# Soham4001A/F16_JSB

Hardware: AMD Instinct MI355X
Metric: env-steps/sec at 65 536 envs, 1/2/4/8 MI355X; HBM GB/s fraction (higher is better)
Workload: dtype f32

## Files before the change

f16_jsb_amd/csrc/f16_device.h:

```cpp
#pragma once
#include <hip/hip_runtime.h>
#include <stdint.h>

#include "../../include/f16env.h"
#include "f16_tables.h"

namespace f16 {

enum DebugBits {
  DBG_STATE_INDEX = 1,
  DBG_WINDOW_POS = 2,
  DBG_DONE_LIST = 4,
  DBG_TABLE_SEGMENT = 8,
  DBG_RESET_INDEX = 16,
  DBG_RING_SLOT = 32,
  DBG_FRAME_INDEX = 64,
};
#ifdef F16_DEBUG_CHECKS
__device__ unsigned int g_f16_violations;
#define F16_CHECK(cond, bit)                                   \
  do {                                                         \
    if (!(cond)) atomicOr(&::f16::g_f16_violations, (bit));    \
  } while (0)
#else
// ... 156 lines not shown
  const float T2 = 2.0f * __builtin_fmaf(q1, q3, -(q0 * q2));
  const float T5 = 2.0f * __builtin_fmaf(q2, q3, q0 * q1);
  const float T8 = __builtin_fmaf(q3, q3, __builtin_fmaf(-q2, q2, __builtin_fmaf(-q1, q1, q0 * q0)));
  const float we = (float)0.00007292115;
  pqr[0] = __builtin_fmaf(-T2, we, wI[0]);
  pqr[1] = __builtin_fmaf(-T5, we, wI[1]);
  pqr[2] = __builtin_fmaf(-T8, we, wI[2]);
}
__device__ __forceinline__ float ground_speed(float vx, float vy, float vz, float rx, float ry, float rz) {
  const float vv = vx * vx + vy * vy + vz * vz;
  const float vr = vx * rx + vy * ry + vz * rz;
  const float rr = rx * rx + ry * ry + rz * rz;
  return __builtin_amdgcn_sqrtf(fmaxf(vv - vr * vr * __builtin_amdgcn_rcpf(rr), 0.0f));
}
__device__ __forceinline__ void latch_from_state(Lane& L) {
  float pqr[3];
  pqr_aero(L.q, L.wI, pqr);
  L.lx[F16L_P_AERO] = pqr[0]; L.lx[F16L_Q_AERO] = pqr[1]; L.lx[F16L_R_AERO] = pqr[2];
  const double w = 0.00007292115;
  L.lx[F16L_VG_FPS] = ground_speed((float)(L.vI[0] + w * L.rI[1]), (float)(L.vI[1] - w * L.rI[0]), (float)L.vI[2],
                                   (float)L.rI[0], (float)L.rI[1], (float)L.rI[2]);
}

template <bool NT = false>
__device__ __forceinline__ void st16(float4* p, float4 v) {
  if (NT) {
    typedef float v4f __attribute__((ext_vector_type(4)));
    __builtin_nontemporal_store(__builtin_bit_cast(v4f, v), reinterpret_cast<v4f*>(p));
  } else {
    *p = v;
  }
}

template <bool GUST>
__device__ __forceinline__ void lane_unpack(const float4 (&c)[NCOL], float4 w, float4 g, Lane& L) {
  L.rI[0] = f2d(c[0].x, c[0].y); L.rI[1] = f2d(c[0].z, c[0].w);
  L.rI[2] = f2d(c[1].x, c[1].y); L.vI[0] = f2d(c[1].z, c[1].w);
  L.vI[1] = f2d(c[2].x, c[2].y); L.vI[2] = f2d(c[2].z, c[2].w);
  L.epa = f2d(c[3].x, c[3].y); L.ep_ret = f2d(c[3].z, c[3].w);
  L.ndv1[0] = c[4].x; L.ndv1[1] = c[4].y; L.ndv1[2] = c[4].z; L.dv2[0] = c[4].w;
  L.dv2[1] = c[5].x; L.dv2[2] = c[5].y; L.aI[0] = c[5].z; L.aI[1] = c[5].w;
  L.aI[2] = c[6].x; L.aIp[0] = c[6].y; L.aIp[1] = c[6].z; L.aIp[2] = c[6].w;
  L.q[0] = c[7].x; L.q[1] = c[7].y; L.q[2] = c[7].z; L.q[3] = c[7].w;
  L.wI[0] = c[8].x; L.wI[1] = c[8].y; L.wI[2] = c[8].z; L.wId[0] = c[8].w;
  L.wId[1] = c[9].x; L.wId[2] = c[9].y; L.ba[0] = 0.0f; L.ba[1] = c[9].z; L.ba[2] = c[9].w;
  L.tef = c[10].x; L.ail = c[10].y; L.ele = c[10].z; L.rud = c[10].w;
  L.lef = c[11].x; L.sb = c[11].y; L.pri = c[11].z; L.prp = c[11].w;
  L.ppi = c[12].x; L.pyi = c[12].y; L.pyp = c[12].z; L.ppp = 0.0f;
  L.n2 = without_sign_flag(c[12].w); L.n1 = 0.0f;
  L.lx[F16L_ALPHA] = c[13].x; L.lx[F16L_BETA] = c[13].y; L.lx[F16L_MACH] = c[13].z; L.lx[F16L_VC_KTS] = c[13].w;
  L.last_d = without_sign_flag(c[14].x); L.step = __float_as_int(c[14].y);
  L.lx[F16L_NPY] = c[14].z; L.lx[F16L_NPZ] = c[14].w;
  L.goal[0] = c[15].x; L.goal[1] = c[15].y; L.goal[2] = c[15].z; L.ep_count = __float_as_int(c[15].w);
  L.flags = (sign_flag(c[12].w) ? LANE_FLAG_AUG : 0) | (sign_flag(c[14].x) ? LANE_FLAG_FRESH : 0);
  latch_from_state(L);
#pragma unroll
  for (int j = 0; j < 3; ++j) {
    L.wst[j] = GUST ? (&w.x)[j] : 0.0f;
    L.gust[j] = GUST ? (&g.x)[j] : 0.0f;
    L.wind[j] = L.wst[j] + L.gust[j];
  }
}
template <bool GUST = false>
__device__ __forceinline__ void lane_fetch(const SoA& s, int64_t k, float4 (&c)[NCOL], float4& w, float4& g) {
  const int64_t n = s.n;
  const float4* p = s.c + k;
#pragma unroll
  for (int j = 0; j < NCOL; ++j, p += n) c[j] = *p;
  w = make_float4(0.f, 0.f, 0.f, 0.f);
  g = w;
  if (GUST) {
    w = *p;
    g = *(p + n);
  }
}
template <bool GUST = false>
__device__ __forceinline__ void lane_load(const SoA& s, int64_t k, Lane& L) {
  float4 c[NCOL], w, g;
  lane_fetch<GUST>(s, k, c, w, g);
  lane_unpack<GUST>(c, w, g, L);
}
__device__ __forceinline__ void lane_load_lds(const float4* cols, Lane& L) {
  float4 c[NCOL];
#pragma unroll
  for (int j = 0; j < NCOL; ++j) c[j] = cols[j];
  const float4 z = make_float4(0.f, 0.f, 0.f, 0.f);
  lane_unpack<false>(c, z, z, L);
}

template <bool GUST = false, int PART = 0, bool NT = false>
__device__ __forceinline__ void lane_store(const SoA& s, int64_t k, const Lane& L, bool with15 = true) {
  const int64_t n = s.n;
  float4 c[NCOL];
  c[0] = make_float4(dlo(L.rI[0]), dhi(L.rI[0]), dlo(L.rI[1]), dhi(L.rI[1]));
  c[1] = make_float4(dlo(L.rI[2]), dhi(L.rI[2]), dlo(L.vI[0]), dhi(L.vI[0]));
  c[2] = make_float4(dlo(L.vI[1]), dhi(L.vI[1]), dlo(L.vI[2]), dhi(L.vI[2]));
  c[3] = make_float4(dlo(L.epa), dhi(L.epa), dlo(L.ep_ret), dhi(L.ep_ret));
  c[4] = make_float4(L.ndv1[0], L.ndv1[1], L.ndv1[2], L.dv2[0]);
  c[5] = make_float4(L.dv2[1], L.dv2[2], L.aI[0], L.aI[1]);
  c[6] = make_float4(L.aI[2], L.aIp[0], L.aIp[1], L.aIp[2]);
  c[7] = make_float4(L.q[0], L.q[1], L.q[2], L.q[3]);
  c[8] = make_float4(L.wI[0], L.wI[1], L.wI[2], L.wId[0]);
  c[9] = make_float4(L.wId[1], L.wId[2], L.ba[1], L.ba[2]);
  c[10] = make_float4(L.tef, L.ail, L.ele, L.rud);
  c[11] = make_float4(L.lef, L.sb, L.pri, L.prp);
  c[12] = make_float4(L.ppi, L.pyi, L.pyp, with_sign_flag(L.n2, (L.flags & LANE_FLAG_AUG) != 0));
// ... 8 lines not shown
      if (j != 15 || with15) st16<NT>(p, c[j]);
  if (GUST && PART != 2) {
    st16<NT>(p, make_float4(L.wst[0], L.wst[1], L.wst[2], 0.0f));
    st16<NT>(p + n, make_float4(L.gust[0], L.gust[1], L.gust[2], 0.0f));
  }
}

struct Seg {
  int i;
  float f;
};
__device__ __forceinline__ float rcpf(float x) { return __builtin_amdgcn_rcpf(x); }
__device__ __forceinline__ float fsqrt(float x) { return __builtin_amdgcn_sqrtf(x); }
__device__ __forceinline__ float fdiv(float a, float b) { return a * __builtin_amdgcn_rcpf(b); }

template <int N>
__device__ __forceinline__ Seg bracket(const float (&bp)[N], const float* pairs, float x) {
#ifdef F16_BRACKET_CMP
  int i = 1;
#pragma unroll
  for (int k = 1; k < N - 1; ++k) i += (bp[k] < x) ? 1 : 0;
#else
  uint32_t c = 0;
#pragma unroll
  for (int k = 1; k < N - 1; ++k) c += __float_as_uint(bp[k] - x) >> 31;
  const int i = 1 + (int)c;
#endif
  F16_CHECK(i >= 1 && i <= N - 1, DBG_TABLE_SEGMENT);
  const float2 p = reinterpret_cast<const float2*>(pairs)[i - 1];
  float f = (x - p.x) * p.y;
  f = __builtin_amdgcn_fmed3f(f, 0.0f, 1.0f);
  return {i, f};
}
template <int N>
__device__ __forceinline__ Seg bracket_guess(const float* pairs, float x, float u) {
  static_assert(N >= 3, "guess bracket needs an interior breakpoint");
  const int g = (int)__builtin_amdgcn_fmed3f(u, 0.0f, (float)(N - 3));
  const float2* P = reinterpret_cast<const float2*>(pairs);
  const float2 p0 = P[g], p1 = P[g + 1];
  const bool up = x > p1.x;
  const float lo = up ? p1.x : p0.x, iv = up ? p1.y : p0.y;
  const int i = g + 1 + (up ? 1 : 0);
  F16_CHECK(i >= 1 && i <= N - 1, DBG_TABLE_SEGMENT);
  float f = (x - lo) * iv;
  f = __builtin_amdgcn_fmed3f(f, 0.0f, 1.0f);
  return {i, f};
}
template <int N>
constexpr double guess_h(const float (&bp)[N]) { return ((double)bp[N - 1] - (double)bp[0]) / (N - 1); }
template <int N>
constexpr bool guess_ok_uniform(const float (&bp)[N]) {
  const double h = guess_h(bp), x0 = (double)bp[0] + 0.5 * h;
  for (int k = 1; k <= N - 3; ++k) {
    const double b = x0 + k * h;
    if (!((double)bp[k] + 1e-5 < b && b < (double)bp[k + 1] - 1e-5)) return false;
  }
  return true;
}
template <int N>
__device__ __forceinline__ Seg bracket_g_uniform(const float (&bp)[N], const float* pairs, float x) {
  const double h = guess_h(bp);
  const float ginv = (float)(1.0 / h), c0 = (float)(-((double)bp[0] + 0.5 * h) / h);
  return bracket_guess<N>(pairs, x, __builtin_fmaf(x, ginv, c0));
}
__device__ __forceinline__ float machu_u(float x) {
  x = fminf(x, 4.0f);
// ... 493 lines not shown
    L.n2 = 60.0f + tp * 40.0f;
    L.n1 = 30.0f + tp * 70.0f;
    L.flags = (aug_cmd > 0.0f) ? (L.flags | LANE_FLAG_AUG) : (L.flags & ~LANE_FLAG_AUG);
  } else {
    const float nn = fminf((L.n2 - 60.0f) * (1.0f / 40.0f) + 0.1f, 1.0f);
    const float u = 1.0f - nn;
    const float spool = (90.0f / 3.36f) * rcpf(1.0f + 3.0f * u * u * u + (1.0f - sigma));
    L.n2 = seekf(L.n2, 60.0f + tp * 40.0f, spool, spool * 3.0f, dt);
    L.n1 = seekf(L.n1, 30.0f + tp * 70.0f, spool, spool * 2.4f, dt);
  }
  const float n2n = (L.n2 - 60.0f) * (1.0f / 40.0f);
  float thrust = idle + mil * n2n * n2n;
  if (!(L.flags & LANE_FLAG_AUG)) thrust *= (1.0f - 0.03f);
  if (aug_cmd > 0.0f) {
    L.flags |= LANE_FLAG_AUG;
    const float tdiff = 29000.0f * ev[2] - thrust;
    thrust += tdiff * aug_cmd;
  } else {
    L.flags &= ~LANE_FLAG_AUG;
  }
  return thrust;
}

struct AeroIn {
  float qbar, alpha, beta, mach, p, q, r, bi2vel, ci2vel, kclge;
  float de, da, dr, dlef, flap, dsb;
};
__device__ __forceinline__ void aero(const AeroIn& a, const float* T, float* F6) {
#ifdef F16_GUESS_BRACKET
  static_assert(guess_ok_uniform(BP_alpha_bp) && guess_ok_uniform(BP_beta13_bp) && machu_guess_ok(),
                "guess-bracket crossings must lie inside their segments");
  const Seg sa = bracket_g_uniform(BP_alpha_bp, T + OFF_pair_alpha, a.alpha);
#else
  const Seg sa = bracket(BP_alpha_bp, T + OFF_pair_alpha, a.alpha);
#endif
  float A[F16_N_A1D];
  {
    const float* r0 = T + (OFF_alpha1d + __umul24((unsigned)(sa.i - 1), 2u * F16_N_A1D));
#pragma unroll
    for (int k = 0; k < F16_N_A1D / 2; ++k) {
      const f2v r = blend2(sa.f, ld2(r0 + 2 * k), ld2(r0 + F16_N_A1D + 2 * k));
      A[2 * k] = r.x;
      A[2 * k + 1] = r.y;
    }
  }
  const Seg se = bracket(BP_de_bp, T + OFF_pair_de, a.de);
  float ADE[3];
  {
    const float* p0 = T + (OFF_ade + __umul24(__umul24((unsigned)(sa.i - 1), F16_N_DE) + (unsigned)(se.i - 1), 6u));
    const float* p1 = p0 + 6;
    const f2v c1 = blend2(sa.f, ld2(p0), ld2(p0 + 2)), c2 = blend2(sa.f, ld2(p1), ld2(p1 + 2));
    const f2v r = blend2(se.f, c1, c2 - c1);
    ADE[0] = r.x; ADE[1] = r.y;
    const f2v t1 = ld2(p0 + 4), t2 = ld2(p1 + 4);
    const float d1 = blend(sa.f, t1.x, t1.y), d2 = blend(sa.f, t2.x, t2.y);
    ADE[2] = d1 + se.f * (d2 - d1);
  }
#ifdef F16_GUESS_BRACKET
  const Seg sb13 = bracket_g_uniform(BP_beta13_bp, T + OFF_pair_beta13, a.beta);
#else
  const Seg sb13 = bracket(BP_beta13_bp, T + OFF_pair_beta13, a.beta);
#endif
  float AB13[2];
  {
    const float* p0 = T + (OFF_ab13 + 4u * (__umul24((unsigned)(sa.i - 1), F16_N_B13) + (unsigned)(sb13.i - 1)));
    const float* p1 = p0 + 4;
    const f2v c1 = blend2(sa.f, ld2(p0), ld2(p0 + 2)), c2 = blend2(sa.f, ld2(p1), ld2(p1 + 2));
    const f2v r = blend2(sb13.f, c1, c2 - c1);
    AB13[0] = r.x; AB13[1] = r.y;
  }
  static_assert(beta7_is_even_beta13(), "beta7 grid must be the even beta13 breakpoints");
  Seg sb7;
  {
    sb7.i = 1 + ((sb13.i - 1) >> 1);
    const float2 p = reinterpret_cast<const float2*>(T + OFF_pair_beta7)[sb7.i - 1];
    sb7.f = __builtin_amdgcn_fmed3f((a.beta - p.x) * p.y, 0.0f, 1.0f);
  }
  float AB7[4];
  {
    const float* p0 = T + (OFF_ab7 + 8u * (__umul24((unsigned)(sa.i - 1), F16_N_B7) + (unsigned)(sb7.i - 1)));
    const float* p1 = p0 + 8;
#pragma unroll
    for (int k = 0; k < 4; k += 2) {
      const f2v c1 = blend2(sa.f, ld2(p0 + k), ld2(p0 + k + 4)), c2 = blend2(sa.f, ld2(p1 + k), ld2(p1 + k + 4));
      const f2v r = blend2(sb7.f, c1, c2 - c1);
      AB7[k] = r.x; AB7[k + 1] = r.y;
    }
  }
#ifdef F16_GUESS_BRACKET
  const Seg sm = bracket_guess<13>(T + OFF_pair_machu, a.mach, machu_u(a.mach));
#else
  const Seg sm = bracket(BP_machu, T + OFF_pair_machu, a.mach);
#endif
  float MU[MACHU_NT];
  {
    const float* r0 = T + (OFF_machu_v + __umul24((unsigned)(sm.i - 1), 2u * MACHU_NT));
#pragma unroll
    for (int k = 0; k + 1 < MACHU_NT; k += 2) {
      const f2v r = blend2(sm.f, ld2(r0 + 2 * k), ld2(r0 + 2 * k + 2));
      MU[k] = r.x; MU[k + 1] = r.y;
    }
    if (MACHU_NT & 1) {
      const f2v t = ld2(r0 + 2 * MACHU_NT - 2);
      MU[MACHU_NT - 1] = blend(sm.f, t.x, t.y);
    }
  }
  const float CDmach = MU[MU_CDmach], CYb_M = MU[MU_CYb_M], Clb_M = MU[MU_Clb_M];
  const float Clda_M = MU[MU_Clda_M], Cldr_M = MU[MU_Cldr_M], Cma_M = MU[MU_Cma_M];
  const float Cnb_M = MU[MU_Cnb_M], Cnda_M = MU[MU_Cnda_M], Cndr_M = MU[MU_Cndr_M];

  const float qS = a.qbar * S_W;
  const float qc = a.q * a.ci2vel, pb = a.p * a.bi2vel, rb = a.r * a.bi2vel;
  const float D = qS * (ADE[ADE_CDDh] + CDmach + a.dlef * A[A1D_CDDlef] + a.flap * 0.08f +
                        0.0f * 0.027f + a.dsb * A[A1D_CDDsb] + qc * A[A1D_CDq] +
                        qc * a.dlef * A[A1D_CDq_Dlef]);
  const float Y = qS * (a.beta * -1.146f + a.beta * CYb_M + a.da * -0.0226f + a.dr * 0.086f +
                        pb * A[A1D_CYp] + rb * A[A1D_CYr]);
  const float Lf = qS * (a.kclge * ADE[ADE_CLDh] + a.dlef * a.kclge * A[A1D_CLDlef] +
                         a.flap * a.kclge * 0.35f + a.kclge * a.dsb * A[A1D_CLDsb] +
                         qc * a.kclge * A[A1D_CLq] + qc * a.dsb * A[A1D_CLq_Dsb]);
  const float qSb = qS * B_W, qSc = qS * CBAR;
  const float Lm = qSb * (AB13[AB13_Clb] + a.beta * Clb_M + pb * A[A1D_Clp] + rb * A[A1D_Clr] +
                          a.da * AB7[AB7_Clda] + a.alpha * a.da * Clda_M + a.alpha * a.dr * Cldr_M +
                          a.dr * AB7[AB7_Cldr]);
  const float Mm = qSc * (ADE[ADE_CmDh] + a.alpha * Cma_M + a.dsb * A[A1D_CmDsb] + qc * A[A1D_Cmq]);
  const float Nm = qSb * (AB13[AB13_Cnb] + a.beta * Cnb_M + pb * A[A1D_Cnp] + rb * A[A1D_Cnr] +
                          a.da * Cnda_M + a.da * AB7[AB7_Cnda] + a.dr * AB7[AB7_Cndr] +
                          a.alpha * a.dr * Cndr_M);
  F6[0] = D; F6[1] = Y; F6[2] = Lf; F6[3] = Lm; F6[4] = Mm; F6[5] = Nm;
}

template <bool LOWREG = false, bool WIND = true>
__device__ __forceinline__ void frame(Lane& L, const float* cmd, double& ce, double& se, const AltRef& A,
                                      const float* T, const ModelConsts& C, bool ic F16_STAMP_ARG) {
  const float dt = C.dt_f;
  const FcsTab tb = fcs_tables(L, T);
  if (!ic) {
    const float hx = C.half_dt * L.wI[0], hy = C.half_dt * L.wI[1], hz = C.half_dt * L.wI[2];
    const float a2 = hx * hx + hy * hy + hz * hz;
    float na2 = __builtin_fmaf(-hz, hz, __builtin_fmaf(-hx, hx, -(hy * hy)));
    if constexpr (!LOWREG) asm("" : "+v"(na2));
    float ca, sa;
    if constexpr (LOWREG) {
      ca = 1.0f - a2 * (0.5f - a2 * (1.0f / 24.0f - a2 * (1.0f / 720.0f - a2 * (1.0f / 40320.0f))));
      sa = 1.0f - a2 * (1.0f / 6.0f - a2 * (1.0f / 120.0f - a2 * (1.0f / 5040.0f - a2 * (1.0f / 362880.0f))));
    } else {
    ca = __builtin_fmaf(na2, __builtin_fmaf(na2, __builtin_fmaf(na2, __builtin_fmaf(na2, 1.0f / 40320.0f,
                                                                                         1.0f / 720.0f),
                                                                       1.0f / 24.0f), 0.5f), 1.0f);
    sa = __builtin_fmaf(na2, __builtin_fmaf(na2, __builtin_fmaf(na2, __builtin_fmaf(na2, 1.0f / 362880.0f,
                                                                                   1.0f / 5040.0f),
                                                                 1.0f / 120.0f), 1.0f / 6.0f), 1.0f);
    }
    if (__builtin_expect(na2 <= -0.25f, 0)) {
      const float ang = fsqrt(-na2);
      float sn;
      sincosf(ang, &sn, &ca);
      sa = sn / ang;
    }
    const float p0 = ca, p1 = hx * sa, p2 = hy * sa, p3 = hz * sa;
    {
      const float q0 = L.q[0], q1 = L.q[1], q2 = L.q[2], q3 = L.q[3];
      const float n0 = q0 * p0 - q1 * p1 - q2 * p2 - q3 * p3;
      const float n1 = q0 * p1 + q1 * p0 + q2 * p3 - q3 * p2;
      const float n2 = q0 * p2 - q1 * p3 + q2 * p0 + q3 * p1;
      const float n3 = q0 * p3 + q1 * p2 - q2 * p1 + q3 * p0;
      const float rn = __builtin_amdgcn_rsqf(n0 * n0 + n1 * n1 + n2 * n2 + n3 * n3);
// ... 21 lines not shown
  derive(L, ce, se, A, d);
  F16_STAMP(stamps, ST_DERIVE);
  float wb[3] = {0.0f, 0.0f, 0.0f};
  if (WIND) mvec(d.Tl2b, L.wind, wb);
  const float ua = d.uvw[0] - wb[0], va = d.uvw[1] - wb[1], wa = d.uvw[2] - wb[2];
  const float muw = ua * ua + wa * wa;
  const float vt = fsqrt(muw + va * va);
  const bool moving = muw > 0.0f;
  const float alpha = fatan2<LOWREG>(moving ? wa : 0.0f, ua);
  const float suw = fsqrt(muw);
  const float beta = fatan2<LOWREG, true>(moving ? va : 0.0f, suw);
  const float iuw = rcpf(suw), ivt = rcpf(vt);
  const float ca_ = moving ? ua * iuw : 1.0f, sa_ = moving ? wa * iuw : 0.0f;
  const float cb_ = moving ? suw * ivt : 1.0f, sb_ = moving ? va * ivt : 0.0f;
  const float inv2v = (vt != 0.0f) ? 0.5f * ivt : 0.0f;
  const float bi2vel = B_W * inv2v, ci2vel = CBAR * inv2v;
  const float vg = d.vg;
  float u1[3], u2[3], u3[3];
  cross_c(MP.eye, L.wId, u1);
  cross_c(MP.eye, L.wI, u2);
  crossf(L.wI, u2, u3);
  const float npy = (L.ba[1] - u1[1] - u3[1]) * C.inv_gref;
  const float npz = (L.ba[2] - u1[2] - u3[2]) * C.inv_gref;
  const float h = (float)d.h_ft;
  const Atm atm = atmosphere(h);
  const float sigma = atm.rho * C.inv_rho_sl;
  const float qbar = 0.5f * atm.rho * vt * vt;
  const float mach = vt * rcpf(atm.a);
  const float down_b[3] = {d.Tl2b[2], d.Tl2b[5], d.Tl2b[8]};
  const float vmac_d = dot3c(MP.rp, down_b);
  const float hbmac = (h - vmac_d) * (1.0f / B_W);
  F16_STAMP(stamps, ST_ATM);
  FcsOut fc;
  fcs_run<LOWREG>(L, cmd, d.Tl2b[8], d.uvw[1], T, tb, C, dt, ic, fc);
  F16_STAMP(stamps, ST_FCS);
  const float thrust = engine_run<LOWREG>(L, fc.throttle, mach, h, sigma, T, dt, ic);
  F16_STAMP(stamps, ST_ENGINE);
  AeroIn ai;
  ai.qbar = qbar; ai.alpha = alpha; ai.beta = beta; ai.mach = mach;
  ai.p = d.pqr[0]; ai.q = d.pqr[1]; ai.r = d.pqr[2];
  ai.bi2vel = bi2vel; ai.ci2vel = ci2vel;
  ai.kclge = tab1_fast_end(BP_kclge, T + OFF_pair_kclge, T + OFF_kclge_vd, hbmac);
  ai.de = fc.de; ai.da = fc.da; ai.dr = fc.dr; ai.dlef = fc.dlef; ai.flap = fc.flap_mix; ai.dsb = fc.dsb;
  float A6[6];
  aero(ai, T, A6);
  const float fw0 = -A6[0], fw1 = A6[1], fw2 = -A6[2];
  float F[3], M[3];
  F[0] = ca_ * cb_ * fw0 - ca_ * sb_ * fw1 - sa_ * fw2;
  F[2] = sa_ * cb_ * fw0 - sa_ * sb_ * fw1 + ca_ * fw2;
  F[1] = sb_ * fw0 + cb_ * fw1;
  float rxF[3];
  cross_c(MP.rp, F, rxF);
  M[0] = A6[3] + rxF[0];
  M[1] = A6[4] + rxF[1];
  M[2] = A6[5] + rxF[2];
  F[0] += thrust;
  if (MP.eng[2] != 0.0f) M[1] += MP.eng[2] * thrust;
  if (MP.eng[1] != 0.0f) M[2] -= MP.eng[1] * thrust;
  F16_STAMP(stamps, ST_AERO);
#pragma unroll
  for (int j = 0; j < 3; ++j) L.ba[j] = F[j] * MP.inv_mass;
  float abI[3];
  mtvec(d.Ti2b, L.ba, abI);
#pragma unroll
  for (int j = 0; j < 3; ++j) L.aI[j] = abI[j] + d.gI[j];
  float Jw[3], wxJw[3], rhs[3];
// ... 15 lines not shown
```

f16_jsb_amd/csrc/f16env.hip:

```cpp
#include <hip/hip_ext.h>
#include <hip/hip_runtime.h>

#include <math.h>
#include <stdint.h>
#include <stdio.h>
#include <stdlib.h>
#include <string.h>

#include <string>
#include <vector>

#include "../../include/f16env.h"
#include "f16_device.h"
#ifndef F16_C15_ALWAYS
#define F16_C15_ALWAYS 0
#endif

using namespace f16;

static thread_local std::string g_err;
static int set_err(int code, const char* msg) {
  g_err = msg;
  return code;
}
// ... 403 lines not shown
#endif
  L.last_d = norm3f(f0[12] - f0[0], f0[13] - f0[1], f0[14] - f0[2]);
}

__device__ __forceinline__ void earth_angle(double epa, double& ce, double& se) {
  if (fabs(epa) < 0.01) {
    const double e2 = epa * epa;
    ce = 1.0 - e2 * (0.5 - e2 * (1.0 / 24.0 - e2 * (1.0 / 720.0 - e2 * (1.0 / 40320.0))));
    se = epa * (1.0 - e2 * (1.0 / 6.0 - e2 * (1.0 / 120.0 - e2 * (1.0 / 5040.0 - e2 * (1.0 / 362880.0)))));
  } else {
    ce = cos(epa);
    se = sin(epa);
  }
}

#ifndef BLOCK
#define BLOCK 256
#endif
#define FRAME_PITCH 16
#ifndef IMG_OFF
#define IMG_OFF 0
#endif

#ifdef F16_ASM_VMCNT
#define VM_DRAIN() asm volatile("s_waitcnt vmcnt(0)" ::: "memory")
#else
#define VM_DRAIN()                          \
  do {                                      \
    asm volatile("" ::: "memory");          \
    __builtin_amdgcn_s_waitcnt(0x0F70);     \
    asm volatile("" ::: "memory");          \
  } while (0)
#endif

__device__ __forceinline__ void dma16(const float* g, float* lds) {
  __builtin_amdgcn_global_load_lds((const void __attribute__((address_space(1)))*)g,
                                   (void __attribute__((address_space(3)))*)lds, 16, 0, 0);
}
__device__ __forceinline__ void dma4(const float* g, float* lds) {
  __builtin_amdgcn_global_load_lds((const void __attribute__((address_space(1)))*)g,
                                   (void __attribute__((address_space(3)))*)lds, 4, 0, 0);
}
__device__ __forceinline__ void stage_tables_issue(float* sT) {
  constexpr int NP = F16_BLOB_FLOATS / 4;
  static_assert(F16_BLOB_FLOATS % 4 == 0, "blob must be whole 16-byte pieces");
  const int wave_base = threadIdx.x & ~63;
#ifdef F16_STAGE_BLOCKDIM
  for (int r = 0; r < NP; r += blockDim.x) {
#else
  for (int r = 0; r < NP; r += BLOCK) {
#endif
    const int piece = r + threadIdx.x;
    if (piece < NP) dma16(F16_BLOB_INIT + 4 * piece, sT + 4 * (r + wave_base));
  }
}
__device__ __forceinline__ void stage_tables(float* sT) {
  stage_tables_issue(sT);
  VM_DRAIN();
  __syncthreads();
}

__device__ __forceinline__ void quat_mul_ref(const float* a, const float* b, float* o) {
#pragma clang fp contract(off)
  const float dot = a[1] * b[1] + a[2] * b[2] + a[3] * b[3];
  o[0] = a[0] * b[0] - dot;
  const float cx = a[2] * b[3] - a[3] * b[2], cy = a[3] * b[1] - a[1] * b[3], cz = a[1] * b[2] - a[2] * b[1];
// ... 76 lines not shown
static constexpr int WFRESH = 16 * 64;
static constexpr int WSTASH = 16 * 64;
static constexpr int WIN_WAVE_FLOATS = WFRESH + WSTASH;

struct StepPre {
  const float4* sc;
  const float* act;
  const float4* tmpl;
  int64_t n;
};
enum { XV_X = 1, XV_FEAT = 2 };
template <int MODE, bool GT = false, bool ROLL = false, bool LOWREG = false, bool WIN = false, bool NT = false,
          bool HALF = false, int XV = 0>
__device__ __forceinline__ void step_body(const StepArgs& a, float* sT_lds, float4* sTmpl, int* sDone, float* dynl,
                                          const StepPre* pre = nullptr) {
  const float* sT = GT ? static_cast<const float*>(F16_BLOB_INIT) : sT_lds;
  constexpr bool GUST = (MODE & 2) != 0, DEFER = MODE != 0;
  constexpr bool SAMPLE = ROLL || (XV & XV_X) != 0;
  constexpr bool FEATW = ROLL || (XV & XV_FEAT) != 0;
  constexpr int EPW = HALF ? 32 : 64;
#ifdef F16_STAMPS
  Stamps stamps = {};
  stamps.last = memtime();
#endif
  if (HALF && a.half_delay > 0 && blockIdx.x >= gridDim.x / 2) {
    const uint64_t t0 = __builtin_amdgcn_s_memtime();
    while (__builtin_amdgcn_s_memtime() - t0 < (uint64_t)a.half_delay) __builtin_amdgcn_s_sleep(8);
  }
  const int KC = a.E.K * F16_OBS_DIM, HC = (a.E.K - 1) * F16_OBS_DIM;
  const int wave = threadIdx.x >> 6, lane = threadIdx.x & 63;
  const int64_t row0 = (int64_t)blockIdx.x * (4 * EPW) + wave * EPW;
  const int64_t nE = pre ? pre->n : a.E.n;
  const int rows = (int)(nE - row0 < EPW ? (nE - row0 > 0 ? nE - row0 : 0) : EPW);
  const bool image = a.lds_image != 0;
  const bool in_step_reset = WIN && DEFER && a.icc.c != nullptr && !(a.E.flags & F16_FLAG_NO_AUTORESET);
#ifdef F16_NO_STASH
  constexpr bool STASH = false;
#else
  constexpr bool STASH = LOWREG && WIN;
#endif
  float* img = dynl + (size_t)wave * image_floats_per_wave(KC);
  auto issue_stack_dma = [&]() {
    if (image && rows > 0) {
      const float* prev = a.obs_prev + row0 * KC;
      const int total = rows * KC;
      const int n16 = total >> 2;
      for (int b = 0; b < n16; b += 64) {
        const int piece = b + lane;
        if (piece < n16) dma16(prev + 4 * piece, img + IMG_OFF + 4 * b);
      }
      if (lane < (total & 3)) dma4(prev + 4 * n16 + lane, img + IMG_OFF + 4 * n16);
    }
  };
  const int64_t k = row0 + lane;
  const bool live = (!HALF || lane < EPW) && k < nE;
  F16_CHECK(rows >= 0 && rows <= 64 && (!live || row0 + lane < nE), DBG_STATE_INDEX);
  if (WIN) F16_CHECK(a.wpos >= a.E.K - 1 && a.wpos >= 0, DBG_WINDOW_POS);
  int done = 0;
  Lane L;
  float4 av = make_float4(0.f, 0.f, 0.f, 0.f);
  if (!GT) stage_tables_issue(sT_lds);
  if (!DEFER && threadIdx.x < NCOL + TMPL_FRAME_COLS)
    dma16(reinterpret_cast<const float*>((pre ? pre->tmpl : a.tmpl.c) + (threadIdx.x < NCOL ? threadIdx.x : threadIdx.x + NCOL_ALL - NCOL)),
          reinterpret_cast<float*>(sTmpl));
  float4 cl[NCOL], wl, gl;
  if (live) {
    if (pre) {
      const SoA sp = {const_cast<float4*>(pre->sc), pre->n};
      lane_fetch<GUST>(sp, k, cl, wl, gl);
      if (!SAMPLE || !a.sample_act) av = reinterpret_cast<const float4*>(pre->act)[k];
    } else {
      lane_fetch<GUST>(a.s, k, cl, wl, gl);
      if (!SAMPLE || !a.sample_act) av = reinterpret_cast<const float4*>(a.act)[k];
    }
  }
  VM_DRAIN();
#ifndef F16_PROLOGUE_NO_SCHED_BARRIER
  __builtin_amdgcn_sched_barrier(0);
#endif
  if (live) lane_unpack<GUST>(cl, wl, gl, L);
  __syncthreads();
  issue_stack_dma();
  if (SAMPLE && a.sample_act && live) av = philox_action(a.act_seed, (uint64_t)(a.E.id_base + k), a.act_step);
  bool fresh = false;
  float* stg = dynl + (size_t)wave * WIN_WAVE_FLOATS;
  if (live) {
    fresh = (L.flags & LANE_FLAG_FRESH) != 0;
    L.flags &= ~LANE_FLAG_FRESH;
  }
  if (WIN && fresh && a.E.K > 1) {
    const float* src = a.wy + k * a.wenv + (int64_t)(a.wpos - 1) * a.wrow;
#pragma unroll
    for (int j = 0; j < 4; ++j) dma16(src + 4 * j, stg + j * 256);
  }
  F16_STAMP(stamps, ST_LOAD);
  float f[F16_OBS_DIM], f0[F16_OBS_DIM];
  float rew_out = 0.0f;
  int flags_out = 0;
  double ce = 1.0, se = 0.0;
  AltRef A;
  if (live) {
    const float4 ac = (ROLL && a.clip_act) ? clip_box(av) : av;
    const float cmd[4] = {ac.x, ac.y, ac.z, ac.w};
    L.step += 1;
    if (GUST) {
      float xi[3];
      rng_normals(a.E.seed, (uint64_t)(a.E.id_base + k), (uint32_t)(L.ep_count - 1), (uint32_t)L.step, xi);
#pragma unroll
      for (int j = 0; j < 3; ++j) {
        L.gust[j] = __builtin_fmaf(a.E.gust_a, L.gust[j], a.E.gust_b * xi[j]);
        L.wind[j] = L.wst[j] + L.gust[j];
      }
    }
    earth_angle(L.epa, ce, se);
    A = alt_ref(L, ce, se);
    F16_STAMP(stamps, ST_ENVPRE);
    float4* stash = reinterpret_cast<float4*>(stg + WFRESH);
    if (STASH) {
      stash[lane] = make_float4(L.goal[0], L.goal[1], L.goal[2], L.last_d);
      stash[64 + lane] = make_float4(__int_as_float(L.step), __int_as_float(L.ep_count), dlo(L.ep_ret), dhi(L.ep_ret));
      stash[128 + lane] = make_float4(dlo(L.epa), dhi(L.epa), GUST ? L.gust[0] : 0.0f, GUST ? L.gust[1] : 0.0f);
      if (GUST) stash[192 + lane] = make_float4(L.gust[2], L.wst[0], L.wst[1], L.wst[2]);
      asm volatile("" ::: "memory");
    }
    for (int s = 0; s < a.E.down_sample; ++s)
      frame<LOWREG, GUST>(L, cmd, ce, se, A, sT, a.C, false F16_STAMP_PASS);
    if (STASH) {
      asm volatile("" ::: "memory");
      const float4 g = stash[lane], e = stash[64 + lane];
      L.goal[0] = g.x; L.goal[1] = g.y; L.goal[2] = g.z; L.last_d = g.w;
      L.step = __float_as_int(e.x); L.ep_count = __float_as_int(e.y); L.ep_ret = f2d(e.z, e.w);
      const float4 w = stash[128 + lane];
      L.epa = f2d(w.x, w.y);
      for (int s = 0; s < a.E.down_sample; ++s) L.epa += a.C.epa_dt;
      if (GUST) {
        const float4 u = stash[192 + lane];
        L.gust[0] = w.z; L.gust[1] = w.w; L.gust[2] = u.x; L.wst[0] = u.y; L.wst[1] = u.z; L.wst[2] = u.w;
      }
    }
  }
  const bool early_store = LOWREG && !a.done_idx;
  if (early_store) {
    VM_DRAIN();
    if (live) lane_store<GUST, 1, NT>(a.s, k, L);
  }
  if (live) {
    make_frame(L, ce, se, A, f);
    F16_STAMP(stamps, ST_FRAME_OBS);
    float r32;
    flags_out = env_reward(L, f, a.E, r32);
    F16_STAMP(stamps, ST_REWARD);
    done = flags_out & 3;
    rew_out = r32;
  }
  if (!early_store) VM_DRAIN();
  if (a.done_idx) {
    const unsigned long long m = __ballot(done);
    if (m) {
      int base = 0;
      if (lane == 0) base = atomicAdd(a.n_done, __popcll(m));
      base = __shfl(base, 0);
      F16_CHECK(base + __popcll(m) <= nE, DBG_DONE_LIST);
      if (done) a.done_idx[base + __popcll(m & ((1ull << lane) - 1ull))] = (int32_t)k;
    }
  }
  if (a.E.flags & F16_FLAG_NAN_GUARD) {
    const unsigned long long qm = __ballot(flags_out & 4);
    if (qm && lane == 0) atomicAdd(a.nonfinite, (unsigned long long)__popcll(qm));
  }
  if (a.E.flags & F16_FLAG_OBS_CHECK) {
    const unsigned long long om = __ballot(live && obs_out_of_bounds(f));
// ... 2241 lines not shown
```

Before: 4.324 billion.

## Split prologue state loads into ordered partial waits and peel first frame

Reorders the per-lane column loads so the columns needed first (position, velocity, quaternion, alpha/mach) are issued early. The code then waits with a partial vmcnt instead of draining all loads, and unpacks the state in three parts, so the late columns (actuator and controller state) are consumed inside the first peeled frame just before the flight-control step. It also adds an optional windowed bracket search that uses a ballot to scan only a sub-range of breakpoints when the whole wave lies inside it. This is meant to hide global-load latency in the prologue, but it depends on correct vmcnt accounting and adds code size and register pressure.

```diff
diff --git a/f16_jsb_amd/csrc/f16_device.h b/f16_jsb_amd/csrc/f16_device.h
--- a/f16_jsb_amd/csrc/f16_device.h
+++ b/f16_jsb_amd/csrc/f16_device.h
@@ -212,33 +212,41 @@
   }
 }
 
-template <bool GUST>
+template <bool GUST, int PART = 0>
 __device__ __forceinline__ void lane_unpack(const float4 (&c)[NCOL], float4 w, float4 g, Lane& L) {
-  L.rI[0] = f2d(c[0].x, c[0].y); L.rI[1] = f2d(c[0].z, c[0].w);
-  L.rI[2] = f2d(c[1].x, c[1].y); L.vI[0] = f2d(c[1].z, c[1].w);
-  L.vI[1] = f2d(c[2].x, c[2].y); L.vI[2] = f2d(c[2].z, c[2].w);
-  L.epa = f2d(c[3].x, c[3].y); L.ep_ret = f2d(c[3].z, c[3].w);
-  L.ndv1[0] = c[4].x; L.ndv1[1] = c[4].y; L.ndv1[2] = c[4].z; L.dv2[0] = c[4].w;
-  L.dv2[1] = c[5].x; L.dv2[2] = c[5].y; L.aI[0] = c[5].z; L.aI[1] = c[5].w;
-  L.aI[2] = c[6].x; L.aIp[0] = c[6].y; L.aIp[1] = c[6].z; L.aIp[2] = c[6].w;
-  L.q[0] = c[7].x; L.q[1] = c[7].y; L.q[2] = c[7].z; L.q[3] = c[7].w;
-  L.wI[0] = c[8].x; L.wI[1] = c[8].y; L.wI[2] = c[8].z; L.wId[0] = c[8].w;
-  L.wId[1] = c[9].x; L.wId[2] = c[9].y; L.ba[0] = 0.0f; L.ba[1] = c[9].z; L.ba[2] = c[9].w;
-  L.tef = c[10].x; L.ail = c[10].y; L.ele = c[10].z; L.rud = c[10].w;
-  L.lef = c[11].x; L.sb = c[11].y; L.pri = c[11].z; L.prp = c[11].w;
-  L.ppi = c[12].x; L.pyi = c[12].y; L.pyp = c[12].z; L.ppp = 0.0f;
-  L.n2 = without_sign_flag(c[12].w); L.n1 = 0.0f;
-  L.lx[F16L_ALPHA] = c[13].x; L.lx[F16L_BETA] = c[13].y; L.lx[F16L_MACH] = c[13].z; L.lx[F16L_VC_KTS] = c[13].w;
-  L.last_d = without_sign_flag(c[14].x); L.step = __float_as_int(c[14].y);
-  L.lx[F16L_NPY] = c[14].z; L.lx[F16L_NPZ] = c[14].w;
-  L.goal[0] = c[15].x; L.goal[1] = c[15].y; L.goal[2] = c[15].z; L.ep_count = __float_as_int(c[15].w);
-  L.flags = (sign_flag(c[12].w) ? LANE_FLAG_AUG : 0) | (sign_flag(c[14].x) ? LANE_FLAG_FRESH : 0);
-  latch_from_state(L);
-#pragma unroll
-  for (int j = 0; j < 3; ++j) {
-    L.wst[j] = GUST ? (&w.x)[j] : 0.0f;
-    L.gust[j] = GUST ? (&g.x)[j] : 0.0f;
-    L.wind[j] = L.wst[j] + L.gust[j];
+  if (PART == 0 || PART == 1) {
+    L.rI[0] = f2d(c[0].x, c[0].y); L.rI[1] = f2d(c[0].z, c[0].w);
+    L.rI[2] = f2d(c[1].x, c[1].y); L.vI[0] = f2d(c[1].z, c[1].w);
+    L.vI[1] = f2d(c[2].x, c[2].y); L.vI[2] = f2d(c[2].z, c[2].w);
+    L.epa = f2d(c[3].x, c[3].y); L.ep_ret = f2d(c[3].z, c[3].w);
+    L.ndv1[0] = c[4].x; L.ndv1[1] = c[4].y; L.ndv1[2] = c[4].z; L.dv2[0] = c[4].w;
+    L.dv2[1] = c[5].x; L.dv2[2] = c[5].y; L.aI[0] = c[5].z; L.aI[1] = c[5].w;
+    L.aI[2] = c[6].x; L.aIp[0] = c[6].y; L.aIp[1] = c[6].z; L.aIp[2] = c[6].w;
+    L.q[0] = c[7].x; L.q[1] = c[7].y; L.q[2] = c[7].z; L.q[3] = c[7].w;
+    L.wI[0] = c[8].x; L.wI[1] = c[8].y; L.wI[2] = c[8].z; L.wId[0] = c[8].w;
+    L.wId[1] = c[9].x; L.wId[2] = c[9].y; L.ba[0] = 0.0f; L.ba[1] = c[9].z; L.ba[2] = c[9].w;
+    L.lx[F16L_ALPHA] = c[13].x; L.lx[F16L_BETA] = c[13].y; L.lx[F16L_MACH] = c[13].z; L.lx[F16L_VC_KTS] = c[13].w;
+    latch_from_state(L);
+  }
+  if (PART == 0 || PART == 2) {
+    L.last_d = without_sign_flag(c[14].x); L.step = __float_as_int(c[14].y);
+    L.lx[F16L_NPY] = c[14].z; L.lx[F16L_NPZ] = c[14].w;
+    L.goal[0] = c[15].x; L.goal[1] = c[15].y; L.goal[2] = c[15].z; L.ep_count = __float_as_int(c[15].w);
+    L.flags = sign_flag(c[14].x) ? LANE_FLAG_FRESH : 0;
+#pragma unroll
+    for (int j = 0; j < 3; ++j) {
+      L.wst[j] = GUST ? (&w.x)[j] : 0.0f;
+      L.gust[j] = GUST ? (&g.x)[j] : 0.0f;
+      L.wind[j] = L.wst[j] + L.gust[j];
+    }
+  }
+  if (PART == 0 || PART == 3) {
+    L.tef = c[10].x; L.ail = c[10].y; L.ele = c[10].z; L.rud = c[10].w;
+    L.lef = c[11].x; L.sb = c[11].y; L.pri = c[11].z; L.prp = c[11].w;
+    L.ppi = c[12].x; L.pyi = c[12].y; L.pyp = c[12].z; L.ppp = 0.0f;
+    L.n2 = without_sign_flag(c[12].w); L.n1 = 0.0f;
+    if (PART == 0) L.flags = (sign_flag(c[12].w) ? LANE_FLAG_AUG : 0) | (sign_flag(c[14].x) ? LANE_FLAG_FRESH : 0);
+    else L.flags |= sign_flag(c[12].w) ? LANE_FLAG_AUG : 0;
   }
 }
 template <bool GUST = false>
@@ -252,6 +260,37 @@
   if (GUST) {
     w = *p;
     g = *(p + n);
+  }
+}
+static constexpr int FETCH_ORDER[NCOL] = {13, 8, 7, 3, 0, 1, 2, 4, 5, 6, 9, 14, 10, 11, 12, 15};
+static constexpr int FETCH_SPLIT = 12;
+constexpr bool fetch_order_is_permutation() {
+  int seen = 0;
+  for (int j = 0; j < NCOL; ++j) seen |= 1 << FETCH_ORDER[j];
+  return seen == (1 << NCOL) - 1 && FETCH_ORDER[NCOL - 1] == 15;
+}
+static_assert(fetch_order_is_permutation(), "FETCH_ORDER must name every column once, C15 last");
+typedef float v4f_t __attribute__((ext_vector_type(4)));
+typedef const v4f_t __attribute__((address_space(1))) * GCol;
+__device__ __forceinline__ float4 fetch_col(GCol p) {
+  const float4 v = __builtin_bit_cast(float4, *p);
+  __builtin_amdgcn_sched_barrier(0);
+  return v;
+}
+template <bool GUST, bool C15_EARLY, int PART>
+__device__ __forceinline__ void lane_fetch_ordered(GCol cols, int64_t n, int64_t k, float4 (&c)[NCOL], float4& w, float4& g) {
+  const GCol p = cols + k;
+#pragma unroll
+  for (int i = PART ? FETCH_SPLIT : 0; i < (PART ? NCOL - (C15_EARLY ? 1 : 0) : FETCH_SPLIT); ++i)
+    c[FETCH_ORDER[i]] = fetch_col(p + FETCH_ORDER[i] * n);
+  if (PART == 0) {
+    if (C15_EARLY) c[15] = fetch_col(p + 15 * n);
+    w = make_float4(0.f, 0.f, 0.f, 0.f);
+    g = w;
+    if (GUST) {
+      w = fetch_col(p + COL_WIND * n);
+      g = fetch_col(p + COL_GUST * n);
+    }
   }
 }
 template <bool GUST = false>
@@ -326,6 +365,38 @@
   f = __builtin_amdgcn_fmed3f(f, 0.0f, 1.0f);
   return {i, f};
 }
+constexpr int bracket_window_const(int n, int klo) {
+  return klo < n - 2 ? (klo > 0 ? klo : 0) : n - 2;
+}
+template <int KLO, int KHI, int N>
+__device__ __forceinline__ Seg bracket_window(const float (&bp)[N], const float* pairs, float x) {
+#if !defined(F16_BRACKET_WINDOW) || defined(F16_BRACKET_FULL)
+  return bracket(bp, pairs, x);
+#else
+  static_assert(0 <= KLO && KLO < KHI && KHI <= N - 1, "window ends must be breakpoints of the grid");
+  uint32_t c;
+  if (__ballot(!(x > bp[KLO] && x <= bp[KHI])) == 0) {
+    c = (uint32_t)bracket_window_const(N, KLO);
+#pragma unroll
+    for (int k = (KLO + 1 > 1 ? KLO + 1 : 1); k < (KHI < N - 1 ? KHI : N - 1); ++k) c += __float_as_uint(bp[k] - x) >> 31;
+  } else {
+    c = 0;
+#pragma unroll
+    for (int k = 1; k < N - 1; ++k) c += __float_as_uint(bp[k] - x) >> 31;
+  }
+  const int i = 1 + (int)c;
+  F16_CHECK(i >= 1 && i <= N - 1, DBG_TABLE_SEGMENT);
+  const float2 p = reinterpret_cast<const float2*>(pairs)[i - 1];
+  float f = (x - p.x) * p.y;
+  f = __builtin_amdgcn_fmed3f(f, 0.0f, 1.0f);
+  return {i, f};
+#endif
+}
+enum { WIN_ALPHA_LO = 0, WIN_ALPHA_HI = 6, WIN_BETA_LO = 4, WIN_BETA_HI = 8, WIN_MACH_LO = 1, WIN_MACH_HI = 7 };
+static_assert(BP_alpha_bp[WIN_ALPHA_LO] == -0.175f && BP_alpha_bp[WIN_ALPHA_HI] == 0.349f, "alpha window (-10, 20] deg");
+static_assert(BP_beta13_bp[WIN_BETA_LO] == -0.175f && BP_beta13_bp[WIN_BETA_HI] == 0.175f, "beta window (-10, 10] deg");
+static_assert(BP_machu[WIN_MACH_LO] == 0.4f && BP_machu[WIN_MACH_HI] == 1.0f, "Mach window (0.4, 1.0]");
+
 template <int N>
 __device__ __forceinline__ Seg bracket_guess(const float* pairs, float x, float u) {
   static_assert(N >= 3, "guess bracket needs an interior breakpoint");
@@ -885,7 +956,7 @@
                 "guess-bracket crossings must lie inside their segments");
   const Seg sa = bracket_g_uniform(BP_alpha_bp, T + OFF_pair_alpha, a.alpha);
 #else
-  const Seg sa = bracket(BP_alpha_bp, T + OFF_pair_alpha, a.alpha);
+  const Seg sa = bracket_window<WIN_ALPHA_LO, WIN_ALPHA_HI>(BP_alpha_bp, T + OFF_pair_alpha, a.alpha);
 #endif
   float A[F16_N_A1D];
   {
@@ -912,7 +983,7 @@
 #ifdef F16_GUESS_BRACKET
   const Seg sb13 = bracket_g_uniform(BP_beta13_bp, T + OFF_pair_beta13, a.beta);
 #else
-  const Seg sb13 = bracket(BP_beta13_bp, T + OFF_pair_beta13, a.beta);
+  const Seg sb13 = bracket_window<WIN_BETA_LO, WIN_BETA_HI>(BP_beta13_bp, T + OFF_pair_beta13, a.beta);
 #endif
   float AB13[2];
   {
@@ -943,7 +1014,7 @@
 #ifdef F16_GUESS_BRACKET
   const Seg sm = bracket_guess<13>(T + OFF_pair_machu, a.mach, machu_u(a.mach));
 #else
-  const Seg sm = bracket(BP_machu, T + OFF_pair_machu, a.mach);
+  const Seg sm = bracket_window<WIN_MACH_LO, WIN_MACH_HI>(BP_machu, T + OFF_pair_machu, a.mach);
 #endif
   float MU[MACHU_NT];
   {
@@ -983,9 +1054,13 @@
   F6[0] = D; F6[1] = Y; F6[2] = Lf; F6[3] = Lm; F6[4] = Mm; F6[5] = Nm;
 }
 
-template <bool LOWREG = false, bool WIND = true>
+struct NoLate {
+  __device__ __forceinline__ void operator()() const {}
+};
+template <bool LOWREG = false, bool WIND = true, class LATE = NoLate>
 __device__ __forceinline__ void frame(Lane& L, const float* cmd, double& ce, double& se, const AltRef& A,
-                                      const float* T, const ModelConsts& C, bool ic F16_STAMP_ARG) {
+                                      const float* T, const ModelConsts& C, bool ic F16_STAMP_ARG,
+                                      const LATE& late = LATE()) {
   const float dt = C.dt_f;
   const FcsTab tb = fcs_tables(L, T);
   if (!ic) {
@@ -1073,6 +1148,10 @@
   const float hbmac = (h - vmac_d) * (1.0f / B_W);
   F16_STAMP(stamps, ST_ATM);
   FcsOut fc;
+  if constexpr (!__is_same(LATE, NoLate)) {
+    __builtin_amdgcn_sched_barrier(0);
+    late();
+  }
   fcs_run<LOWREG>(L, cmd, d.Tl2b[8], d.uvw[1], T, tb, C, dt, ic, fc);
   F16_STAMP(stamps, ST_FCS);
   const float thrust = engine_run<LOWREG>(L, fc.throttle, mach, h, sigma, T, dt, ic);
diff --git a/f16_jsb_amd/csrc/f16env.hip b/f16_jsb_amd/csrc/f16env.hip
--- a/f16_jsb_amd/csrc/f16env.hip
+++ b/f16_jsb_amd/csrc/f16env.hip
@@ -459,6 +459,13 @@
     asm volatile("" ::: "memory");          \
   } while (0)
 #endif
+#define VM_WAIT(k)                                                                      \
+  do {                                                                                  \
+    static_assert((k) >= 0 && (k) < 64, "vmcnt is a 6-bit count");                      \
+    asm volatile("" ::: "memory");                                                      \
+    __builtin_amdgcn_s_waitcnt(0x0F70 | ((k) & 15) | ((((k) >> 4) & 3) << 14));         \
+    asm volatile("" ::: "memory");                                                      \
+  } while (0)
 
 __device__ __forceinline__ void dma16(const float* g, float* lds) {
   __builtin_amdgcn_global_load_lds((const void __attribute__((address_space(1)))*)g,
@@ -601,7 +608,12 @@
   const int64_t row0 = (int64_t)blockIdx.x * (4 * EPW) + wave * EPW;
   const int64_t nE = pre ? pre->n : a.E.n;
   const int rows = (int)(nE - row0 < EPW ? (nE - row0 > 0 ? nE - row0 : 0) : EPW);
-  const bool image = a.lds_image != 0;
+#ifdef F16_PROLOGUE_ONE_WAIT
+  constexpr bool ONE_WAIT = true;
+#else
+  constexpr bool ONE_WAIT = ROLL || (XV & XV_X) != 0;
+#endif
+  const bool image = (ONE_WAIT || !WIN) && a.lds_image != 0;
   const bool in_step_reset = WIN && DEFER && a.icc.c != nullptr && !(a.E.flags & F16_FLAG_NO_AUTORESET);
 #ifdef F16_NO_STASH
   constexpr bool STASH = false;
@@ -633,66 +645,80 @@
     dma16(reinterpret_cast<const float*>((pre ? pre->tmpl : a.tmpl.c) + (threadIdx.x < NCOL ? threadIdx.x : threadIdx.x + NCOL_ALL - NCOL)),
           reinterpret_cast<float*>(sTmpl));
   float4 cl[NCOL], wl, gl;
-  if (live) {
-    if (pre) {
-      const SoA sp = {const_cast<float4*>(pre->sc), pre->n};
-      lane_fetch<GUST>(sp, k, cl, wl, gl);
-      if (!SAMPLE || !a.sample_act) av = reinterpret_cast<const float4*>(pre->act)[k];
-    } else {
-      lane_fetch<GUST>(a.s, k, cl, wl, gl);
-      if (!SAMPLE || !a.sample_act) av = reinterpret_cast<const float4*>(a.act)[k];
-    }
-  }
-  VM_DRAIN();
+  const bool load_act = !SAMPLE || !a.sample_act;
+  constexpr bool C15_EARLY = GUST || STASH;
+  if constexpr (ONE_WAIT) {
+    if (live) {
+      if (pre) {
+        const SoA sp = {const_cast<float4*>(pre->sc), pre->n};
+        lane_fetch<GUST>(sp, k, cl, wl, gl);
+        if (load_act) av = reinterpret_cast<const float4*>(pre->act)[k];
+      } else {
+        lane_fetch<GUST>(a.s, k, cl, wl, gl);
+        if (load_act) av = reinterpret_cast<const float4*>(a.act)[k];
+      }
+    }
+    VM_DRAIN();
 #ifndef F16_PROLOGUE_NO_SCHED_BARRIER
-  __builtin_amdgcn_sched_barrier(0);
+    __builtin_amdgcn_sched_barrier(0);
 #endif
-  if (live) lane_unpack<GUST>(cl, wl, gl, L);
-  __syncthreads();
-  issue_stack_dma();
+    if (live) lane_unpack<GUST>(cl, wl, gl, L);
+    __syncthreads();
+  } else {
+    {
+      float4* scp = pre ? const_cast<float4*>(pre->sc) : a.s.c;
+      const float* actp = pre ? pre->act : a.act;
+      asm volatile("" : "+s"(scp), "+s"(actp));
+      const GCol scg = (GCol)scp, actg = (GCol)actp;
+      const int64_t kc = k < nE ? k : (nE > 0 ? nE - 1 : 0);
+      lane_fetch_ordered<GUST, C15_EARLY, 0>(scg, pre ? pre->n : a.s.n, kc, cl, wl, gl);
+      if (load_act) av = fetch_col(actg + kc);
+      lane_fetch_ordered<GUST, C15_EARLY, 1>(scg, pre ? pre->n : a.s.n, kc, cl, wl, gl);
+    }
+    asm volatile("" ::: "memory");
+    __builtin_amdgcn_sched_barrier(0);
+    if (!GT || !DEFER) VM_WAIT(NCOL + (GUST ? 2 : 0) - (SAMPLE ? 1 : 0));
+    __syncthreads();
+    __builtin_amdgcn_sched_barrier(0);
+    lane_unpack<GUST, 1>(cl, wl, gl, L);
+  }
+  if constexpr (ONE_WAIT) issue_stack_dma();
   if (SAMPLE && a.sample_act && live) av = philox_action(a.act_seed, (uint64_t)(a.E.id_base + k), a.act_step);
+  double ce = 1.0, se = 0.0;
+  AltRef A;
+  if constexpr (!ONE_WAIT) {
+    earth_angle(L.epa, ce, se);
+    A = alt_ref(L, ce, se);
+    __builtin_amdgcn_sched_barrier(0);
+    lane_unpack<GUST, 2>(cl, wl, gl, L);
+  }
   bool fresh = false;
   float* stg = dynl + (size_t)wave * WIN_WAVE_FLOATS;
-  if (live) {
-    fresh = (L.flags & LANE_FLAG_FRESH) != 0;
+  if constexpr (ONE_WAIT) {
+    if (live) {
+      fresh = (L.flags & LANE_FLAG_FRESH) != 0;
+      L.flags &= ~LANE_FLAG_FRESH;
+    }
+  } else {
+    fresh = live && (L.flags & LANE_FLAG_FRESH) != 0;
     L.flags &= ~LANE_FLAG_FRESH;
   }
-  if (WIN && fresh && a.E.K > 1) {
-    const float* src = a.wy + k * a.wenv + (int64_t)(a.wpos - 1) * a.wrow;
-#pragma unroll
-    for (int j = 0; j < 4; ++j) dma16(src + 4 * j, stg + j * 256);
-  }
+  const auto issue_fresh_dma = [&]() {
+    if (WIN && fresh && a.E.K > 1) {
+      const float* src = a.wy + k * a.wenv + (int64_t)(a.wpos - 1) * a.wrow;
+#pragma unroll
+      for (int j = 0; j < 4; ++j) dma16(src + 4 * j, stg + j * 256);
+    }
+  };
+  if constexpr (ONE_WAIT) issue_fresh_dma();
   F16_STAMP(stamps, ST_LOAD);
   float f[F16_OBS_DIM], f0[F16_OBS_DIM];
   float rew_out = 0.0f;
   int flags_out = 0;
-  double ce = 1.0, se = 0.0;
-  AltRef A;
-  if (live) {
-    const float4 ac = (ROLL && a.clip_act) ? clip_box(av) : av;
-    const float cmd[4] = {ac.x, ac.y, ac.z, ac.w};
-    L.step += 1;
-    if (GUST) {
-      float xi[3];
-      rng_normals(a.E.seed, (uint64_t)(a.E.id_base + k), (uint32_t)(L.ep_count - 1), (uint32_t)L.step, xi);
-#pragma unroll
-      for (int j = 0; j < 3; ++j) {
-        L.gust[j] = __builtin_fmaf(a.E.gust_a, L.gust[j], a.E.gust_b * xi[j]);
-        L.wind[j] = L.wst[j] + L.gust[j];
-      }
-    }
-    earth_angle(L.epa, ce, se);
-    A = alt_ref(L, ce, se);
-    F16_STAMP(stamps, ST_ENVPRE);
-    float4* stash = reinterpret_cast<float4*>(stg + WFRESH);
-    if (STASH) {
-      stash[lane] = make_float4(L.goal[0], L.goal[1], L.goal[2], L.last_d);
-      stash[64 + lane] = make_float4(__int_as_float(L.step), __int_as_float(L.ep_count), dlo(L.ep_ret), dhi(L.ep_ret));
-      stash[128 + lane] = make_float4(dlo(L.epa), dhi(L.epa), GUST ? L.gust[0] : 0.0f, GUST ? L.gust[1] : 0.0f);
-      if (GUST) stash[192 + lane] = make_float4(L.gust[2], L.wst[0], L.wst[1], L.wst[2]);
-      asm volatile("" ::: "memory");
-    }
-    for (int s = 0; s < a.E.down_sample; ++s)
+  float cmd[4] = {0.0f, 0.0f, 0.0f, 0.0f};
+  float4* stash = reinterpret_cast<float4*>(stg + WFRESH);
+  const auto rest_frames = [&](int s0) {
+    for (int s = s0; s < a.E.down_sample; ++s)
       frame<LOWREG, GUST>(L, cmd, ce, se, A, sT, a.C, false F16_STAMP_PASS);
     if (STASH) {
       asm volatile("" ::: "memory");
@@ -706,6 +732,55 @@
         const float4 u = stash[192 + lane];
         L.gust[0] = w.z; L.gust[1] = w.w; L.gust[2] = u.x; L.wst[0] = u.y; L.wst[1] = u.z; L.wst[2] = u.w;
       }
+    }
+  };
+#ifdef F16_PROLOGUE_NO_PEEL
+  const int peeled = 0;
+#else
+  const int peeled = (!ONE_WAIT && a.E.down_sample > 0) ? 1 : 0;
+#endif
+  const auto pre_frames = [&]() {
+    const float4 ac = (ROLL && a.clip_act) ? clip_box(av) : av;
+    cmd[0] = ac.x; cmd[1] = ac.y; cmd[2] = ac.z; cmd[3] = ac.w;
+    L.step += 1;
+    if (GUST) {
+      float xi[3];
+      rng_normals(a.E.seed, (uint64_t)(a.E.id_base + k), (uint32_t)(L.ep_count - 1), (uint32_t)L.step, xi);
+#pragma unroll
+      for (int j = 0; j < 3; ++j) {
+        L.gust[j] = __builtin_fmaf(a.E.gust_a, L.gust[j], a.E.gust_b * xi[j]);
+        L.wind[j] = L.wst[j] + L.gust[j];
+      }
+    }
+    if constexpr (ONE_WAIT) {
+      earth_angle(L.epa, ce, se);
+      A = alt_ref(L, ce, se);
+    }
+    F16_STAMP(stamps, ST_ENVPRE);
+    if (STASH) {
+      stash[lane] = make_float4(L.goal[0], L.goal[1], L.goal[2], L.last_d);
+      stash[64 + lane] = make_float4(__int_as_float(L.step), __int_as_float(L.ep_count), dlo(L.ep_ret), dhi(L.ep_ret));
+      stash[128 + lane] = make_float4(dlo(L.epa), dhi(L.epa), GUST ? L.gust[0] : 0.0f, GUST ? L.gust[1] : 0.0f);
+      if (GUST) stash[192 + lane] = make_float4(L.gust[2], L.wst[0], L.wst[1], L.wst[2]);
+      asm volatile("" ::: "memory");
+    }
+  };
+  if constexpr (ONE_WAIT) {
+    if (live) {
+      pre_frames();
+      rest_frames(0);
+    }
+  } else {
+    pre_frames();
+    const auto late = [&]() { lane_unpack<GUST, 3>(cl, wl, gl, L); };
+    if (peeled)
+      frame<LOWREG, GUST>(L, cmd, ce, se, A, sT, a.C, false F16_STAMP_PASS, late);
+    else
+      late();
+    if constexpr (!WIN) issue_stack_dma();
+    if (live) {
+      issue_fresh_dma();
+      rest_frames(peeled);
     }
   }
   const bool early_store = LOWREG && !a.done_idx;
```

New measurement: 4.404 billion, median of 6. +1.8%, better.
